# Trippasch/CudaRayTracer

Measured on AMD Instinct MI355X. Metric: Mray/s (and ms/frame) at 1920x1080, 64 spp, depth 8, random-spheres, higher is better.
Workload: dtype f32; 1 GPU; c2: 1920x1080, 64 spp, depth 8, RTIOW final random-spheres scene; width=1920, height=1080, spp=64, depth=8, parallelism=1 GPU, kernel_variant=-1

## Files before the change

### cudaraytracer_amd/_lib.py

```python
from __future__ import annotations

import ctypes as C
import os

from . import abi

LIB_PATH = _IN_TREE = os.path.join(os.path.dirname(os.path.abspath(__file__)), "librt_hip.so")
LIB_PATH = os.environ.get("RT_HIP_LIB", LIB_PATH)

EXPORTED = [
    "LaunchKernel",
    "LaunchRandInit",
    "LaunchRenderInit",
    "rt_last_error",
    "rt_version",
    "rt_abi_version",
    "rt_set_launch_flags",
    "rt_set_device",
    "rt_scene_create",
    "rt_scene_from_reference_graph",
    "rt_scene_update_materials",
    "rt_scene_destroy",
    "rt_scene_get_info",
    "rt_render_init",
# ... 34 lines not shown
    "rt_set_variant",
    "rt_set_tuning",
    "rt_glibc_srand",
    "rt_glibc_rand_next",
    "rt_builtin_scene",
    "rt_camera_inputs",
    "rt_procedural_texture",
    "rt_reference_graph_flatten",
    "rt_build_host_tables",
    "rt_tile_entries_host",
    "rt_set_tile_occlusion",
    "rt_tile_entries_device",
    "rt_set_bounce_entries",
    "rt_bounce_entries_host",
    "rt_bounce_entry_cells",
]

_lib = None


class RTError(RuntimeError):
    pass


def _declare(lib: C.CDLL) -> None:
    P = C.POINTER
    vp = C.c_void_p
    lib.rt_last_error.restype = C.c_char_p
    lib.rt_version.restype = C.c_char_p
    lib.rt_set_launch_flags.argtypes = [C.c_uint32]
# ... 58 lines not shown
                                               P(C.c_uint32), P(abi.ImageDesc), P(C.c_uint32)]
    lib.rt_build_host_tables.argtypes = [P(abi.SceneDesc), P(C.c_float), P(C.c_float), P(C.c_float),
                                         P(C.c_int32), P(abi.HostTablesInfo)]
    if LIB_PATH == _IN_TREE or hasattr(lib, "rt_tile_entries_host"):
        lib.rt_tile_entries_host.argtypes = [P(abi.SceneDesc), P(abi.InputStruct), C.c_uint32, C.c_uint32, P(abi.Tiling),
                                             C.c_uint32, C.c_uint32, C.c_uint32, P(C.c_uint32)]
    if LIB_PATH == _IN_TREE or hasattr(lib, "rt_set_tile_occlusion"):
        lib.rt_set_tile_occlusion.argtypes = [C.c_int]
        lib.rt_tile_entries_device.argtypes = [vp, P(abi.InputStruct), C.c_uint32, C.c_uint32, P(abi.Tiling), C.c_uint32,
                                               vp, vp]
    if LIB_PATH == _IN_TREE or hasattr(lib, "rt_set_bounce_entries"):
        lib.rt_set_bounce_entries.argtypes = [C.c_int]
        lib.rt_bounce_entries_host.argtypes = [P(abi.SceneDesc), P(C.c_float), P(C.c_float), P(C.c_uint32), P(C.c_uint32),
                                               P(C.c_uint16), P(abi.BounceEntriesInfo)]
        lib.rt_bounce_entry_cells.argtypes = [P(abi.BounceEntriesInfo), P(C.c_float), C.c_uint32, P(C.c_uint32)]
    lib.LaunchKernel.argtypes = [vp, C.c_uint, C.c_uint, C.c_uint, C.c_uint, vp, vp, abi.InputStruct]
    lib.LaunchKernel.restype = None
    lib.LaunchRandInit.argtypes = [vp]
    lib.LaunchRandInit.restype = None
    lib.LaunchRenderInit.argtypes = [abi.Dim3, abi.Dim3, C.c_uint, C.c_uint, vp]
    lib.LaunchRenderInit.restype = None


def lib() -> C.CDLL:
    global _lib
    if _lib is None:
        if not os.path.exists(LIB_PATH):
            raise RTError(f"{LIB_PATH} is missing: build it with `python -c 'import __graft_entry__ as g; g.build()'`")
        handle = C.CDLL(LIB_PATH)
        _declare(handle)
# ... 9 lines not shown
```

### cudaraytracer_amd/abi.py

```python
from __future__ import annotations

import ctypes as C

import numpy as np

RT_SPHERE, RT_XYRECT, RT_XZRECT, RT_YZRECT = 0, 1, 2, 3
RT_LAMBERTIAN, RT_METAL, RT_DIELECTRIC, RT_DIFFUSELIGHT = 0, 1, 2, 3
RT_CONSTANT, RT_CHECKER, RT_IMAGE = 0, 1, 2

RT_FLAG_FAITHFUL_GRID = 1 << 0
RT_FLAG_NO_STATE_WRITEBACK = 1 << 1
RT_FLAG_ACCUMULATE = 1 << 2
RT_FLAG_RIUS_LEFT_TO_RIGHT = 1 << 3
RT_FLAG_COUNT_TESTS = 1 << 4
RT_FLAG_RNG_PHILOX = 1 << 5
RT_FLAG_STATE_SOA = 1 << 6
RT_FLAG_ACCUMULATE_RESET = 1 << 7
RT_CAMERA_JITTER_PHILOX = 1 << 0
RT_DENOISE_DEMODULATE = 1 << 0
RT_DENOISE_COLOR_IS_SUM = 1 << 1
RT_TEMPORAL_COLOR_IS_SUM = 1 << 0
RT_TEMPORAL_RESET = 1 << 1
ABI_VERSION = 14
MOTION_NO_HISTORY = (0.0, 0.0, 0.0, 0.0)
# ... 318 lines not shown
        ("device_bytes", C.c_uint64),
    ]


class HostTablesInfo(C.Structure):
    _fields_ = [("num_nodes", C.c_uint32), ("num_prims", C.c_uint32), ("num_materials", C.c_uint32),
                ("depth", C.c_uint32)]


class BounceEntriesInfo(C.Structure):
    _fields_ = [("num_nodes", C.c_uint32), ("num_chain_nodes", C.c_uint32), ("num_records", C.c_uint32),
                ("depth", C.c_uint32), ("grid_dim", C.c_uint32 * 3), ("grid_origin", C.c_float * 3),
                ("grid_inv", C.c_float * 3), ("grid_off", C.c_float * 3)]


class GlibcRand(C.Structure):
    _fields_ = [("r", C.c_int32 * 34), ("idx", C.c_uint32)]


STATE_WORDS = 12
assert C.sizeof(CurandState) == 48
assert C.sizeof(InputStruct) == 72
assert C.sizeof(HittableDesc) == 40
assert C.sizeof(MaterialDesc) == 48
assert C.sizeof(TextureDesc) == 32


def make_inputs(origin, orientation, up, far_plane, near_plane, fov, bg_start, bg_end) -> InputStruct:
    s = InputStruct()
    s.origin[:] = [float(v) for v in origin]
# ... 13 lines not shown
```

### cudaraytracer_amd/csrc/api.cpp

```cpp
#include <hip/hip_runtime_api.h>

#include <algorithm>
#include <atomic>
#include <chrono>
#include <cmath>
#include <new>
#include <stdexcept>
#include <cstring>
#include <mutex>
#include <unordered_set>

#include "../../include/rt_reference_graph.h"
#include "rt_bounce_entry.h"
#include "rt_internal.h"
#include "rt_scene_device.h"

namespace rt {

static thread_local std::string g_last_error;

void set_error(const std::string& msg) { g_last_error = msg; }

template <class F>
static int guarded(const char* what, F&& f) {
// ... 33 lines not shown
    if (s->nodes48) (void)hipFree((void*)s->nodes48);
    if (s->refs) (void)hipFree((void*)s->refs);
    s->nodes48 = s->refs = nullptr;
    if (s->prims) (void)hipFree((void*)s->prims);
    if (s->prims_flat) (void)hipFree((void*)s->prims_flat);
    if (s->ref_nodes) (void)hipFree((void*)s->ref_nodes);
    if (s->flat_boxes) (void)hipFree((void*)s->flat_boxes);
    if (s->flat_ref_pairs) (void)hipFree((void*)s->flat_ref_pairs);
    s->prims_flat = s->ref_nodes = s->flat_boxes = s->flat_ref_pairs = nullptr;
    if (s->bvh_ref_nodes) (void)hipFree((void*)s->bvh_ref_nodes);
    if (s->bvh_boxes) (void)hipFree((void*)s->bvh_boxes);
    if (s->bvh_ref_pairs) (void)hipFree((void*)s->bvh_ref_pairs);
    s->bvh_ref_nodes = s->bvh_boxes = s->bvh_ref_pairs = nullptr;
    if (s->leaf_records) (void)hipFree((void*)s->leaf_records);
    if (s->bounce_grid) (void)hipFree((void*)s->bounce_grid);
    s->leaf_records = s->bounce_grid = nullptr;
    if (s->prim_source) (void)hipFree((void*)s->prim_source);
    if (s->flat_source) (void)hipFree((void*)s->flat_source);
    s->prim_source = s->flat_source = nullptr;
    if (s->mats) (void)hipFree((void*)s->mats);
    if (s->imgs) (void)hipFree((void*)s->imgs);
    s->nodes = s->prims = s->mats = nullptr;
    s->imgs = nullptr;
    s->texels = nullptr;
}

int create_device_scene(const HostScene& h, rt_scene** out, std::shared_ptr<void> shared_texels) {
    rt_scene* s = new rt_scene();
    s->host = h;
    s->host.texels = std::vector<uint8_t>();
    DeviceScene& d = s->dev;
// ... 19 lines not shown
    if ((rc = upload(h.flat_boxes, &p, "hipMalloc/hipMemcpy(flat_boxes)"))) goto fail;
    d.flat_boxes = p;
    if ((rc = upload(h.bvh_ref_nodes, &p, "hipMalloc/hipMemcpy(bvh_ref_nodes)"))) goto fail;
    d.bvh_ref_nodes = p;
    if ((rc = upload(h.bvh_boxes, &p, "hipMalloc/hipMemcpy(bvh_boxes)"))) goto fail;
    d.bvh_boxes = p;
    if ((rc = upload(h.bvh_ref_pairs, &p, "hipMalloc/hipMemcpy(bvh_ref_pairs)"))) goto fail;
    d.bvh_ref_pairs = p;
    d.flat_runs[0] = h.flat_runs[0];
    d.flat_runs[1] = h.flat_runs[1];
    if (!h.bounce_grid.empty()) {
        if ((rc = upload(h.leaf_records, &p, "hipMalloc/hipMemcpy(leaf_records)"))) goto fail;
        d.leaf_records = p;
        if ((rc = upload(h.bounce_grid, &p, "hipMalloc/hipMemcpy(bounce_grid)"))) goto fail;
        d.bounce_grid = p;
        for (int i = 0; i < 3; i++) {
            d.grid_dim[i] = h.grid_dim[i];
            d.grid_inv[i] = h.grid_inv[i];
            d.grid_off[i] = h.grid_off[i];
        }
    }
    if ((rc = upload(h.prim_source, &p, "hipMalloc/hipMemcpy(prim_source)"))) goto fail;
    d.prim_source = p;
    if ((rc = upload(h.flat_source, &p, "hipMalloc/hipMemcpy(flat_source)"))) goto fail;
    d.flat_source = p;
    if ((rc = upload(h.mats, &p, "hipMalloc/hipMemcpy(materials)"))) goto fail;
    d.mats = p;
    if ((rc = upload(h.imgs, &p, "hipMalloc/hipMemcpy(images)"))) goto fail;
    d.imgs = p;
    if (shared_texels) {
// ... 1 lines not shown
    } else {
        if ((rc = upload(h.texels, &p, "hipMalloc/hipMemcpy(texels)"))) goto fail;
        if (p) s->texel_block = std::shared_ptr<void>(p, [](void* q) { (void)hipFree(q); });
    }
    d.texels = s->texel_block.get();
    d.num_nodes = h.num_nodes;
    d.num_prims = h.num_prims;
    d.num_mats = h.num_mats;
    d.num_imgs = (uint32_t)(h.imgs.size() / 4);
    d.depth = h.depth;
    d.has_image_textures = h.has_image_textures;
    d.has_textures = h.has_textures;
    d.has_rects = h.has_rects;
    d.device_bytes = (h.nodes.size() + h.nodes48.size() + h.refs.size() + h.prims.size() + h.prims_flat.size() + h.ref_nodes.size() +
                      h.flat_boxes.size() + h.flat_ref_pairs.size() + h.bvh_ref_nodes.size() + h.bvh_boxes.size() + h.bvh_ref_pairs.size() + h.mats.size() +
                      h.prim_source.size() + h.flat_source.size() + h.leaf_records.size()) * 4 + h.bounce_grid.size() * 2 +
                     h.imgs.size() * 4 + h.texels.size();
    *out = s;
    return RT_OK;
fail:
    free_device(&d);
    delete s;
    return rc;
}

static void keep_description(rt_scene** scene, const rt_scene_desc& d, int texel_bytes) {
    static const uint8_t kHasData = 0;
    rt_scene* s = *scene;
    try {
        s->materials.assign(d.materials, d.materials + d.num_materials);
        s->images.assign(d.images, d.images + d.num_images);
// ... 121 lines not shown

struct ImageKey {
    const void* data;
    int32_t width, height;
    bool operator==(const ImageKey& o) const { return data == o.data && width == o.width && height == o.height; }
};

struct LaunchEntry {
    int device = 0;
    const void* world = nullptr;
    uint64_t last_use = 0;
    std::vector<rt_hittable_desc> hittables;
    std::vector<rt_material_desc> materials;
    std::vector<ImageKey> images;
    int texel_bytes = 0;
    std::shared_ptr<rt_scene> scene;
};

std::shared_ptr<rt_scene> own_scene(rt_scene* s, int device) {
    return std::shared_ptr<rt_scene>(s, [device](rt_scene* p) {
        int cur = 0;
        const bool restore = hipGetDevice(&cur) == hipSuccess;
        (void)hipSetDevice(device);
        rt_scene_destroy(p);
        if (restore) (void)hipSetDevice(cur);
    });
}

constexpr size_t kLaunchCacheEntries = 8;
std::mutex g_launch_mu;
// ... 24 lines not shown
        for (LaunchEntry& c : g_launch_cache)
            if (c.device == device && c.world == world) ent = &c;
        if (!ent) {
            if (g_launch_cache.size() >= kLaunchCacheEntries) {
                auto lru = std::min_element(g_launch_cache.begin(), g_launch_cache.end(),
                                            [](const LaunchEntry& a, const LaunchEntry& b) { return a.last_use < b.last_use; });
                g_launch_cache.erase(lru);
            }
            g_launch_cache.emplace_back();
            ent = &g_launch_cache.back();
            ent->device = device;
            ent->world = world;
        }
        ent->last_use = ++g_launch_clock;
        const bool geometry = !ent->scene || !same_bytes(ent->hittables, f.hittables) ||
                              ent->materials.size() != f.materials.size();
        const int texel_bytes = g_texel_bytes == 4 ? 4 : 3;
        const bool new_images = !ent->scene || !(ent->images == images) || ent->texel_bytes != texel_bytes;
        if (geometry || new_images) {
            rt_scene_desc d = f.desc();
            HostScene h;
            r = build_host_scene(&d, &h, &err, new_images);
            if (r) { set_error("LaunchKernel: " + err); return r; }
            rt_scene* fresh = nullptr;
            r = create_device_scene(h, &fresh, new_images ? nullptr : ent->scene->texel_block);
            if (r) return r;
            ent->scene = own_scene(fresh, device);
            ent->texel_bytes = texel_bytes;
        } else if (!same_bytes(ent->materials, f.materials)) {
            r = rt_scene_update_materials(ent->scene.get(), f.materials.data(), (uint32_t)f.materials.size());
            if (r) return r;
        }
        ent->hittables.swap(f.hittables);
        ent->materials.swap(f.materials);
        ent->images.swap(images);
        *out = ent->scene;
        return RT_OK;
    });
    if (host_ms) *host_ms = std::chrono::duration<double, std::milli>(std::chrono::steady_clock::now() - t0).count();
    return rc;
}

}
// ... 139 lines not shown
    });
    if (rc) return rc;
    std::memset(info, 0, sizeof(*info));
    info->num_nodes = h.num_nodes;
    info->depth = h.depth;
    if (h.bounce_grid.empty()) return RT_OK;
    info->num_chain_nodes = h.num_chain_nodes;
    info->num_records = (uint32_t)(h.leaf_records.size() / 4);
    for (int i = 0; i < 3; i++) {
        info->grid_dim[i] = h.grid_dim[i];
        info->grid_origin[i] = h.grid_origin[i];
        info->grid_inv[i] = h.grid_inv[i];
        info->grid_off[i] = h.grid_off[i];
    }
    if (chain_nodes) std::copy(h.chain_nodes.begin(), h.chain_nodes.end(), chain_nodes);
    if (nodes48) std::copy(h.nodes48.begin(), h.nodes48.end(), nodes48);
    if (refs) std::copy(h.refs.begin(), h.refs.end(), refs);
    if (records) std::copy(h.leaf_records.begin(), h.leaf_records.end(), records);
    if (grid) std::copy(h.bounce_grid.begin(), h.bounce_grid.end(), grid);
    return RT_OK;
}

int rt_bounce_entry_cells(const rt_bounce_entries_info* info, const float* origins, uint32_t n, uint32_t* cells) {
    if (!info || (n && (!origins || !cells))) { set_error("rt_bounce_entry_cells: NULL argument"); return RT_ERR_INVALID_ARGUMENT; }
    if (info->num_records == 0 || !info->grid_dim[0] || !info->grid_dim[1] || !info->grid_dim[2]) {
        set_error("rt_bounce_entry_cells: the scene has no bounce-entry table");
        return RT_ERR_INVALID_ARGUMENT;
    }
    const float dimf[3] = {(float)(info->grid_dim[0] - 1u), (float)(info->grid_dim[1] - 1u), (float)(info->grid_dim[2] - 1u)};
    for (uint32_t i = 0; i < n; i++)
        cells[i] = bounce_cell(origins[3 * (size_t)i], origins[3 * (size_t)i + 1], origins[3 * (size_t)i + 2], info->grid_inv,
                               info->grid_off, dimf, info->grid_dim);
    return RT_OK;
}

static TemporalCamera temporal_camera(const rt_input_struct& in) {
    TemporalCamera c;
    const float* up = in.up;
    const float* fw = in.orientation;
    const float cx = up[1] * fw[2] - up[2] * fw[1];
    const float cy = -(up[0] * fw[2] - up[2] * fw[0]);
    const float cz = up[0] * fw[1] - up[1] * fw[0];
    const float inv = 1.0f / std::sqrt((cx * cx + cy * cy) + cz * cz);
    c.right[0] = inv * cx;
    c.right[1] = inv * cy;
    c.right[2] = inv * cz;
    c.fov = in.fov;
// ... 232 lines not shown
```

### cudaraytracer_amd/csrc/render.hip

```cpp
#include <hip/hip_runtime.h>

#include <cfloat>
#include <cstdio>
#include <cstdlib>
#include <cstring>
#include <atomic>
#include <map>
#include <numeric>
#include <memory>
#include <mutex>
#include <tuple>
#include <type_traits>
#include <vector>

#include "rt_epilogue.h"
#include "rt_internal.h"
#include "rt_scene_device.h"
#include "rt_tile_entry.h"

namespace rt {
namespace dev {

struct f3 {
    float x, y, z;
};

enum NodeLayout { NODES_48 = 0, NODES_64 = 2 };
__device__ __forceinline__ f3 mk(float x, float y, float z) { return f3{x, y, z}; }
__device__ __forceinline__ f3 add(f3 a, f3 b) { return mk(a.x + b.x, a.y + b.y, a.z + b.z); }
__device__ __forceinline__ f3 sub(f3 a, f3 b) { return mk(a.x - b.x, a.y - b.y, a.z - b.z); }
__device__ __forceinline__ f3 mulv(f3 a, f3 b) { return mk(a.x * b.x, a.y * b.y, a.z * b.z); }
__device__ __forceinline__ f3 scale(float t, f3 v) { return mk(t * v.x, t * v.y, t * v.z); }
// ... 170 lines not shown
    uint32_t prefetch_stop;
    uint32_t group_tiles;
    uint32_t queue_base;
    uint32_t group_perm_a;
    uint32_t group_perm_b, group_perm_k;
    uint32_t queue_host_reset;
    uint32_t linger_ticks;
    uint32_t group_chunk;
    const uint4* tile_entries;
    uint32_t camera_resolve;
    uint32_t path_end_step;
    const uint4* bounce_records;
    const uint16_t* bounce_grid;
    float grid_inv[3], grid_off[3];
    float grid_max[3];
    uint32_t grid_nx, grid_ny;
};

constexpr int kStackMax = 64;
constexpr int kBlock = 256;
constexpr uint32_t kQueueCounters = 16;
constexpr uint32_t kQueueSlotWords = kQueueCounters + 3;
static_assert(kQueueCounters >= 1 && kQueueCounters <= 32, "queue heads");
constexpr uint32_t kQueueAllDone = kQueueCounters == 32 ? 0xffffffffu : (1u << kQueueCounters) - 1u;

enum StackKind { STACK_SCRATCH = 0, STACK_LDS = 1, STACK_LDS16 = 3, STACK_NONE = 4 };

struct ScratchStack {
    int s[kStackMax];
    int n;
    __device__ __forceinline__ void init(uint32_t*) { n = 0; }
// ... 1225 lines not shown
                const uint32_t e[6] = {ry & 0xffffu, ry >> 16, rz & 0xffffu, rz >> 16, rw & 0xffffu, rw >> 16};
                uint32_t n = 0;
#pragma unroll
                for (int i = 0; i < 6; i++)
                    if (e[i] != kTileEntryNone) {
                        stk[(kStackBase + i) * 64] = (typename RefW<WIDE>::Entry)e[i];
                        n = (uint32_t)i + 1u;
                    }
                c.sp = kStackBase + n;
            }
        }
    }
}

template <bool WIDE>
__device__ __forceinline__ void v3_bounce_entry(KParamsC* q, typename RefW<WIDE>::Entry* const stk, const f3 ro, Cursor& c) {
    if constexpr (!WIDE) {
        const uint4* const recs = q->bounce_records;
        if (!recs) return;
        const float fx = fminf(fmaxf(__builtin_fmaf(ro.x, q->grid_inv[0], q->grid_off[0]), 0.0f), q->grid_max[0]);
        const float fy = fminf(fmaxf(__builtin_fmaf(ro.y, q->grid_inv[1], q->grid_off[1]), 0.0f), q->grid_max[1]);
        const float fz = fminf(fmaxf(__builtin_fmaf(ro.z, q->grid_inv[2], q->grid_off[2]), 0.0f), q->grid_max[2]);
        const uint32_t cell = ((uint32_t)fz * q->grid_ny + (uint32_t)fy) * q->grid_nx + (uint32_t)fx;
        const uint4 r = recs[q->bounce_grid[cell]];
        const uint32_t e0 = r.x & 0xffffu;
        if (e0 != kTileEntryRoot) {
            c.leaf = (int)e0;
            c.node = (int)(r.x >> 16);
            const uint32_t e[6] = {r.y & 0xffffu, r.y >> 16, r.z & 0xffffu, r.z >> 16, r.w & 0xffffu, r.w >> 16};
            uint32_t n = 0;
#pragma unroll
            for (int i = 0; i < 6; i++) n += e[i] != kTileEntryNone ? 1u : 0u;
#pragma unroll
            for (int i = 0; i < 6; i++)
                if ((uint32_t)i < n) stk[(kStackBase + n - 1u - (uint32_t)i) * 64] = (typename RefW<WIDE>::Entry)e[i];
            c.sp = kStackBase + n;
        }
    }
}
// ... 641 lines not shown
                    c.mode = MODE_ENDED;
                } else if (ended) {
                    col = mk(__uint_as_float(park[(PK_COL + 0) * 64]), __uint_as_float(park[(PK_COL + 1) * 64]),
                             __uint_as_float(park[(PK_COL + 2) * 64]));
                    v3_next_sample<WIDE>(P, x, g, contrib, rng, col, att, sample, depth, ro, rd, c, rays, tile, stk);
                    park[(PK_COL + 0) * 64] = __float_as_uint(col.x);
                    park[(PK_COL + 1) * 64] = __float_as_uint(col.y);
                    park[(PK_COL + 2) * 64] = __float_as_uint(col.z);
                } else {
                    v3_start_trace<WIDE>(P.num_nodes, c, rays);
                    bounce = true;
                    if (COUNT_TESTS && P.ray_dump) dump_ray(P, depth == P.ray_dump_depth, ro, rd);
                }
                v3_park<COMPACT, false>(park, rng, col, att, sample, depth, rays);
            }
            if (bounce) v3_bounce_entry<WIDE>(kparams_reload(), stk, ro, c);
            if (!RT_REPLAY_SAME_PASS || __ballot(c.mode == MODE_REPLAY) == 0u) break;
            bvh_replay_wave(kparams_reload(), prims, c, ro, rd, cnt, COUNT_TESTS);
        }
        if constexpr (kItemsBuild) {
            const uint64_t needm = __ballot(c.mode == MODE_NEED);
            if (items && needm != 0) {
                const uint32_t item = next_item +
                    __builtin_amdgcn_mbcnt_hi((uint32_t)(needm >> 32), __builtin_amdgcn_mbcnt_lo((uint32_t)needm, 0u));
                next_item += (uint32_t)__popcll(needm);
                if (c.mode == MODE_NEED) {
                    if (item < n_items) {
                        const uint32_t p = item & 63u;
                        const uint32_t bx = tile % P.tiles_x, by = tile / P.tiles_x;
                        const uint32_t px = bx * 8u + (p & 7u), pg = global_row(P, by * 8u + (p >> 3));
                        R rng = begin_rng<R>(nullptr, 0u, pg * P.width + px);
// ... 2669 lines not shown
                           (const float*)S.prims, F, E.rec, P.num_tiles);
        rc = hip_check(hipGetLastError(), "rt_render: tile entry kernel launch", RT_ERR_LAUNCH);
        if (rc != RT_OK) return rc;
        E.filled = true;
        E.scene_uid = S.uid;
        E.frame = F;
    }
    P.tile_entries = (const uint4*)E.rec;
    P.camera_resolve = g_camera_resolve == 1 ? kCameraResolveCap : (uint32_t)g_camera_resolve;
    P.path_end_step = (uint32_t)g_path_end_step;
    return RT_OK;
}

void bind_bounce_entries(dev::KParams& P, const int kernel, const DeviceScene& S) {
    if (kernel != 3 || S.wide_refs || !g_bounce_entries || !S.leaf_records || !S.bounce_grid) return;
    P.bounce_records = (const uint4*)S.leaf_records;
    P.bounce_grid = (const uint16_t*)S.bounce_grid;
    for (int i = 0; i < 3; i++) {
        P.grid_inv[i] = S.grid_inv[i];
        P.grid_off[i] = S.grid_off[i];
        P.grid_max[i] = (float)(S.grid_dim[i] - 1u);
    }
    P.grid_nx = S.grid_dim[0];
    P.grid_ny = S.grid_dim[1];
}

void fill_kernel_params(dev::KParams& P, const Variant& V, const LaunchShape& L, const DeviceScene& S) {
    P.lds_wave_words = L.wave_words;
    if (V.kernel == 5 || V.kernel == 6) fill_flat_tables(P, S);
    const int rius_trips = V.kernel == 6 ? g_rius_trips_persistent : g_rius_trips;
    P.rius_cap = rius_trips > 0 ? (uint32_t)rius_trips : 0xffffffffu;
    const uint32_t tile = V.block == 64 ? 8u : 16u;
    P.tiles_x = (P.width + tile - 1) / tile;
    P.num_tiles = P.tiles_x * ((P.local_rows + tile - 1) / tile);
}

// ... 182 lines not shown
```

### cudaraytracer_amd/csrc/rt_bounce_entry.h

```cpp
#pragma once

#include <cmath>
#include <cstdint>

#include "rt_tile_entry.h"

namespace rt {

constexpr uint32_t kBounceGridMaxCells = 4096;
constexpr uint32_t kBounceChainMax = 7;

RT_TILE_HD inline uint32_t bounce_cell(const float x, const float y, const float z, const float* inv, const float* off,
                                       const float* dimf, const uint32_t* dim) {
    const float fx = fminf(fmaxf(fmaf(x, inv[0], off[0]), 0.0f), dimf[0]);
    const float fy = fminf(fmaxf(fmaf(y, inv[1], off[1]), 0.0f), dimf[1]);
    const float fz = fminf(fmaxf(fmaf(z, inv[2], off[2]), 0.0f), dimf[2]);
    return ((uint32_t)fz * dim[1] + (uint32_t)fy) * dim[0] + (uint32_t)fx;
}

}
```

### cudaraytracer_amd/csrc/rt_internal.h

```cpp
#pragma once

#include <cstdint>
#include <string>
#include <vector>

#include "../../include/rt_hip.h"

namespace rt {

constexpr int kLeafMax = 4;
constexpr uint32_t kOccupancyDepth = 12;
extern thread_local int g_leaf_max;
extern thread_local int g_sah_traversal_x10;
extern thread_local int g_texel_bytes;
constexpr int kRegStackDepth = 24;
constexpr uint32_t kFlatMaxPrims = 64;
constexpr uint32_t kRefTreeMaxDepth = 14;
constexpr uint32_t kRefTreeMaxDepthBvh = 31;

struct HostScene {
    std::vector<float> nodes;
    std::vector<float> nodes48;
    std::vector<uint32_t> refs;
    bool wide_refs = false;
// ... 14 lines not shown
    std::vector<float> ref_nodes;
    std::vector<float> flat_ref_pairs;
    std::vector<float> flat_boxes;
    uint32_t flat_runs[2] = {0u, 0u};
    std::vector<float> bvh_ref_nodes;
    std::vector<float> bvh_boxes;
    std::vector<float> bvh_ref_pairs;
    uint32_t num_chain_nodes = 0;
    std::vector<float> chain_nodes;
    std::vector<uint32_t> leaf_records;
    std::vector<uint16_t> bounce_grid;
    uint32_t grid_dim[3] = {0u, 0u, 0u};
    float grid_origin[3] = {0.0f, 0.0f, 0.0f};
    float grid_inv[3] = {0.0f, 0.0f, 0.0f};
    float grid_off[3] = {0.0f, 0.0f, 0.0f};
};

int build_host_scene(const rt_scene_desc* desc, HostScene* out, std::string* err, bool with_texels = true);

int pack_materials(const rt_material_desc* mats, uint32_t n, uint32_t num_images, std::vector<float>* out,
                   std::string* err);

struct FlatDesc {
    std::vector<rt_hittable_desc> hittables;
    std::vector<rt_material_desc> materials;
    std::vector<rt_image_desc> images;
    rt_scene_desc desc() const {
        rt_scene_desc d;
        d.hittables = hittables.data();
        d.num_hittables = (uint32_t)hittables.size();
        d.materials = materials.data();
// ... 69 lines not shown
```

### cudaraytracer_amd/csrc/rt_scene_device.h

```cpp
#pragma once

#include <cstdint>
#include <memory>

#include "rt_internal.h"

namespace rt {

struct DeviceScene {
    const void* nodes = nullptr;
    const void* nodes48 = nullptr;
    const void* refs = nullptr;
    bool wide_refs = false;
    const void* prims = nullptr;
    const void* prims_flat = nullptr;
    const void* ref_nodes = nullptr;
    const void* flat_ref_pairs = nullptr;
    const void* flat_boxes = nullptr;
    const void* bvh_ref_nodes = nullptr;
    const void* bvh_boxes = nullptr;
    const void* bvh_ref_pairs = nullptr;
    uint32_t flat_runs[2] = {0u, 0u};
    const void* prim_source = nullptr;
    const void* flat_source = nullptr;
    const void* leaf_records = nullptr;
    const void* bounce_grid = nullptr;
    uint32_t grid_dim[3] = {0u, 0u, 0u};
    float grid_inv[3] = {0.0f, 0.0f, 0.0f}, grid_off[3] = {0.0f, 0.0f, 0.0f};
    const void* mats = nullptr;
    const void* imgs = nullptr;
    const void* texels = nullptr;
    uint32_t num_nodes = 0, num_prims = 0, num_mats = 0, depth = 0;
    uint32_t num_imgs = 0;
    bool has_image_textures = false;
    bool has_textures = false;
    bool has_rects = false;
    uint64_t device_bytes = 0;
    uint64_t uid = 0;
};

int create_device_scene(const HostScene& h, rt_scene** out, std::shared_ptr<void> shared_texels = nullptr);
// ... 17 lines not shown
```

### cudaraytracer_amd/csrc/scene_build.cpp

```cpp
#include <algorithm>
#include <limits>
#include <functional>
#include <array>
#include <cmath>
#include <cstring>
#include <numeric>

#include "rt_bounce_entry.h"
#include "rt_internal.h"

namespace rt {
namespace {

struct Box {
    float lo[3], hi[3];
    void empty() {
        for (int i = 0; i < 3; i++) { lo[i] = INFINITY; hi[i] = -INFINITY; }
    }
    void grow(const Box& b) {
        for (int i = 0; i < 3; i++) { lo[i] = std::min(lo[i], b.lo[i]); hi[i] = std::max(hi[i], b.hi[i]); }
    }
    float area() const {
        float dx = hi[0] - lo[0], dy = hi[1] - lo[1], dz = hi[2] - lo[2];
        if (!(dx >= 0) || !(dy >= 0) || !(dz >= 0)) return 0.0f;
        return 2.0f * (dx * dy + dy * dz + dz * dx);
    }
// ... 342 lines not shown
                    float d2 = 0.0f;
                    for (int i = 0; i < 3; i++) {
                        const float d = std::max(std::max(b.lo[i] - c[i], c[i] - b.hi[i]), 0.0f);
                        d2 += d * d;
                    }
                    const float area = b.area();
                    if (d2 < best_dist || (d2 == best_dist && area < best_area)) {
                        best = l;
                        best_dist = d2;
                        best_area = area;
                    }
                }
                out->bounce_grid[((size_t)z * dim[1] + y) * dim[0] + x] = (uint16_t)best;
            }

    out->num_chain_nodes = (uint32_t)chain.size();
    out->chain_nodes.resize(chain.size() * 16);
    out->nodes48.resize((size_t)(N + chain.size()) * 12);
    out->refs.resize((size_t)N + chain.size());
    for (size_t i = 0; i < chain.size(); i++) {
        pack_node16(chain[i], out->chain_nodes.data() + i * 16);
        pack_node48(chain[i], false, out->nodes48.data() + (N + i) * 12);
        out->refs[N + i] = ((uint32_t)chain[i].child[0] & 0xffffu) | ((uint32_t)chain[i].child[1] << 16);
    }
    out->leaf_records.resize(records.size() * 4);
    for (size_t i = 0; i < records.size(); i++)
        for (int w = 0; w < 4; w++) out->leaf_records[4 * i + w] = records[i][2 * w] | (records[i][2 * w + 1] << 16);
}

struct RefNode {
    float lo[3], hi[3];
    int child[2];
    uint32_t depth;
};
void ref_prim_box(const rt_hittable_desc& h, float lo[3], float hi[3]) {
    if (h.type == RT_SPHERE) {
// ... 393 lines not shown
```

### cudaraytracer_amd/renderer.py

```python
from __future__ import annotations

import ctypes as C

import numpy as np
import torch

from . import abi
from ._lib import RTError, check, lib
from .scenes import Scene


class DeviceScene:

    def __init__(self, scene: Scene | None = None, reference_graph: int | None = None):
        L = lib()
        self.handle = C.c_void_p()
        self.scene = scene
        if reference_graph is not None:
            check(L.rt_scene_from_reference_graph(C.c_void_p(reference_graph), C.byref(self.handle)),
                  "rt_scene_from_reference_graph")
        else:
            self._desc = scene.desc()
            check(L.rt_scene_create(C.byref(self._desc), C.byref(self.handle)), "rt_scene_create")

# ... 103 lines not shown
            lib().rt_scene_destroy(self.handle)
            self.handle = C.c_void_p()

    def __del__(self):
        try:
            self.close()
        except Exception:
            pass


def set_tile_occlusion(on: bool) -> bool:
    prev = lib().rt_set_tile_occlusion(1 if on else 0)
    if prev < 0:
        check(prev, "rt_set_tile_occlusion")
    return bool(prev)


def camera_rays(inputs: abi.InputStruct, width: int, height: int, pixels=None, jitter=(0.5, 0.5), sample: int = 0,
                seed: int = 1984, frame: int = 0, tiling: abi.Tiling | None = None, device=None):
    if pixels is not None and not isinstance(pixels, torch.Tensor):
        pixels = torch.from_numpy(np.array(pixels, dtype=np.int64).astype(np.uint32).view(np.int32)).cuda()
    if pixels is not None:
        if pixels.dtype not in (torch.int32, torch.uint32) or pixels.dim() != 1 or not pixels.is_cuda:
            raise ValueError("pixels must be a 32-bit integer (n,) tensor on the device")
        pixels = pixels.contiguous()
        device = pixels.device
    elif device is None:
        device = torch.device("cuda", torch.cuda.current_device())
    t = tiling if tiling is not None else abi.Tiling(max(height, 1), 1, 0, height)
    n = pixels.shape[0] if pixels is not None else t.local_rows * width
# ... 335 lines not shown
```

### include/rt_hip.h

```cpp
#ifndef RT_HIP_H
#define RT_HIP_H

#include <stddef.h>
#include <stdint.h>

#ifdef __cplusplus
extern "C" {
#endif

typedef enum rt_status {
    RT_OK = 0,
    RT_ERR_INVALID_ARGUMENT = -1,
    RT_ERR_INVALID_SCENE = -2,
    RT_ERR_OUT_OF_MEMORY = -3,
    RT_ERR_DEVICE = -4,
    RT_ERR_LAUNCH = -5,
    RT_ERR_UNSUPPORTED = -6
} rt_status;

typedef enum rt_hittable_type {
    RT_SPHERE = 0,
    RT_XYRECT = 1,
    RT_XZRECT = 2,
    RT_YZRECT = 3
// ... 427 lines not shown
                           const rt_tiling* tiling, uint32_t flags, void* records, rt_stream stream);

int rt_set_bounce_entries(int on);

typedef struct rt_bounce_entries_info {
    uint32_t num_nodes, num_chain_nodes, num_records, depth;
    uint32_t grid_dim[3];
    float grid_origin[3];
    float grid_inv[3];
    float grid_off[3];
} rt_bounce_entries_info;
int rt_bounce_entries_host(const rt_scene_desc* desc, float* chain_nodes, float* nodes48, uint32_t* refs,
                           uint32_t* records, uint16_t* grid, rt_bounce_entries_info* info);
int rt_bounce_entry_cells(const rt_bounce_entries_info* info, const float* origins, uint32_t n, uint32_t* cells);

typedef struct rt_glibc_rand { int32_t r[34]; uint32_t idx; } rt_glibc_rand;
void rt_glibc_srand(rt_glibc_rand* g, uint32_t seed);
int32_t rt_glibc_rand_next(rt_glibc_rand* g);

int rt_builtin_scene(int which, uint32_t seed, rt_hittable_desc* hittables, uint32_t* num_hittables,
                     rt_material_desc* materials, uint32_t* num_materials);

int rt_procedural_texture(int kind, int32_t width, int32_t height, uint8_t* rgb);

void rt_camera_inputs(const float position[3], const float orientation[3], const float world_up[3],
                      float fov_degrees, float near_plane, float far_plane, const float bg_start[3],
                      const float bg_end[3], rt_input_struct* out);

#ifdef __cplusplus
}
// ... 4 lines not shown
```

Baseline: 34950 Mray/s.

## Add direction-classed bounce entry records to prune unreachable BVH siblings

Extends the bounce-entry grid so each grid record has 25 variants, keyed by the secondary ray's dominant axis and octant, plus a fallback class. On the host, sibling subtrees along the leaf path that a ray in a given direction class cannot reach from the record's region are dropped, and new chain nodes are built from the remaining pairs. The goal is to shorten the restart stack for secondary bounces and so skip box tests. In exchange, each bounce entry now computes the direction class, the record table is 25 times larger, scene build does more work, and the conservative reachability test must stay correct.

Result: faster. 35660 Mray/s (median of 6 runs) (+2.0%).

```diff
diff --git a/cudaraytracer_amd/_lib.py b/cudaraytracer_amd/_lib.py
--- a/cudaraytracer_amd/_lib.py
+++ b/cudaraytracer_amd/_lib.py
@@ -72,6 +72,8 @@
     "rt_set_bounce_entries",
     "rt_bounce_entries_host",
     "rt_bounce_entry_cells",
+    "rt_set_bounce_classes",
+    "rt_bounce_class_entries_host",
 ]
 
 _lib = None
@@ -160,6 +162,11 @@
         lib.rt_bounce_entries_host.argtypes = [P(abi.SceneDesc), P(C.c_float), P(C.c_float), P(C.c_uint32), P(C.c_uint32),
                                                P(C.c_uint16), P(abi.BounceEntriesInfo)]
         lib.rt_bounce_entry_cells.argtypes = [P(abi.BounceEntriesInfo), P(C.c_float), C.c_uint32, P(C.c_uint32)]
+    if LIB_PATH == _IN_TREE or hasattr(lib, "rt_set_bounce_classes"):
+        lib.rt_set_bounce_classes.argtypes = [C.c_int]
+        lib.rt_bounce_class_entries_host.argtypes = [P(abi.SceneDesc), C.c_int, C.c_uint32, P(C.c_uint32), P(C.c_float),
+                                                     P(C.c_uint32), P(C.c_double), P(C.c_float), P(C.c_float), C.c_uint32,
+                                                     P(C.c_uint32), P(abi.BounceClassInfo)]
     lib.LaunchKernel.argtypes = [vp, C.c_uint, C.c_uint, C.c_uint, C.c_uint, vp, vp, abi.InputStruct]
     lib.LaunchKernel.restype = None
     lib.LaunchRandInit.argtypes = [vp]
diff --git a/cudaraytracer_amd/abi.py b/cudaraytracer_amd/abi.py
--- a/cudaraytracer_amd/abi.py
+++ b/cudaraytracer_amd/abi.py
@@ -356,6 +356,15 @@
                 ("grid_inv", C.c_float * 3), ("grid_off", C.c_float * 3)]
 
 
+BOUNCE_CLASSES = 25
+BOUNCE_CLASS_FULL = 24
+
+
+class BounceClassInfo(C.Structure):
+    _fields_ = [("form", C.c_uint32), ("num_records", C.c_uint32), ("num_class_nodes", C.c_uint32),
+                ("first_class_node", C.c_uint32)]
+
+
 class GlibcRand(C.Structure):
     _fields_ = [("r", C.c_int32 * 34), ("idx", C.c_uint32)]
 
diff --git a/cudaraytracer_amd/csrc/api.cpp b/cudaraytracer_amd/csrc/api.cpp
--- a/cudaraytracer_amd/csrc/api.cpp
+++ b/cudaraytracer_amd/csrc/api.cpp
@@ -71,7 +71,8 @@
     s->bvh_ref_nodes = s->bvh_boxes = s->bvh_ref_pairs = nullptr;
     if (s->leaf_records) (void)hipFree((void*)s->leaf_records);
     if (s->bounce_grid) (void)hipFree((void*)s->bounce_grid);
-    s->leaf_records = s->bounce_grid = nullptr;
+    if (s->class_records) (void)hipFree((void*)s->class_records);
+    s->leaf_records = s->bounce_grid = s->class_records = nullptr;
     if (s->prim_source) (void)hipFree((void*)s->prim_source);
     if (s->flat_source) (void)hipFree((void*)s->flat_source);
     s->prim_source = s->flat_source = nullptr;
@@ -121,6 +122,8 @@
         d.leaf_records = p;
         if ((rc = upload(h.bounce_grid, &p, "hipMalloc/hipMemcpy(bounce_grid)"))) goto fail;
         d.bounce_grid = p;
+        if ((rc = upload(h.class_records, &p, "hipMalloc/hipMemcpy(class_records)"))) goto fail;
+        d.class_records = p;
         for (int i = 0; i < 3; i++) {
             d.grid_dim[i] = h.grid_dim[i];
             d.grid_inv[i] = h.grid_inv[i];
@@ -152,7 +155,7 @@
     d.has_rects = h.has_rects;
     d.device_bytes = (h.nodes.size() + h.nodes48.size() + h.refs.size() + h.prims.size() + h.prims_flat.size() + h.ref_nodes.size() +
                       h.flat_boxes.size() + h.flat_ref_pairs.size() + h.bvh_ref_nodes.size() + h.bvh_boxes.size() + h.bvh_ref_pairs.size() + h.mats.size() +
-                      h.prim_source.size() + h.flat_source.size() + h.leaf_records.size()) * 4 + h.bounce_grid.size() * 2 +
+                      h.prim_source.size() + h.flat_source.size() + h.leaf_records.size() + h.class_records.size()) * 4 + h.bounce_grid.size() * 2 +
                      h.imgs.size() * 4 + h.texels.size();
     *out = s;
     return RT_OK;
@@ -304,6 +307,7 @@
     std::vector<rt_material_desc> materials;
     std::vector<ImageKey> images;
     int texel_bytes = 0;
+    int bounce_classes = 0;
     std::shared_ptr<rt_scene> scene;
 };
 
@@ -358,7 +362,7 @@
         }
         ent->last_use = ++g_launch_clock;
         const bool geometry = !ent->scene || !same_bytes(ent->hittables, f.hittables) ||
-                              ent->materials.size() != f.materials.size();
+                              ent->materials.size() != f.materials.size() || ent->bounce_classes != g_bounce_classes;
         const int texel_bytes = g_texel_bytes == 4 ? 4 : 3;
         const bool new_images = !ent->scene || !(ent->images == images) || ent->texel_bytes != texel_bytes;
         if (geometry || new_images) {
@@ -371,6 +375,7 @@
             if (r) return r;
             ent->scene = own_scene(fresh, device);
             ent->texel_bytes = texel_bytes;
+            ent->bounce_classes = g_bounce_classes;
         } else if (!same_bytes(ent->materials, f.materials)) {
             r = rt_scene_update_materials(ent->scene.get(), f.materials.data(), (uint32_t)f.materials.size());
             if (r) return r;
@@ -540,8 +545,9 @@
         info->grid_off[i] = h.grid_off[i];
     }
     if (chain_nodes) std::copy(h.chain_nodes.begin(), h.chain_nodes.end(), chain_nodes);
-    if (nodes48) std::copy(h.nodes48.begin(), h.nodes48.end(), nodes48);
-    if (refs) std::copy(h.refs.begin(), h.refs.end(), refs);
+    const size_t total = (size_t)h.num_nodes + h.num_chain_nodes;
+    if (nodes48) std::copy(h.nodes48.begin(), h.nodes48.begin() + total * 12, nodes48);
+    if (refs) std::copy(h.refs.begin(), h.refs.begin() + total, refs);
     if (records) std::copy(h.leaf_records.begin(), h.leaf_records.end(), records);
     if (grid) std::copy(h.bounce_grid.begin(), h.bounce_grid.end(), grid);
     return RT_OK;
@@ -557,6 +563,64 @@
     for (uint32_t i = 0; i < n; i++)
         cells[i] = bounce_cell(origins[3 * (size_t)i], origins[3 * (size_t)i + 1], origins[3 * (size_t)i + 2], info->grid_inv,
                                info->grid_off, dimf, info->grid_dim);
+    return RT_OK;
+}
+
+int rt_set_bounce_classes(int form) {
+    if (form < 0 || form > 2) {
+        set_error("rt_set_bounce_classes: the value must be 0, 1 or 2");
+        return RT_ERR_INVALID_ARGUMENT;
+    }
+    const int prev = g_bounce_classes;
+    g_bounce_classes = form;
+    return prev;
+}
+
+int rt_bounce_class_entries_host(const rt_scene_desc* desc, int form, uint32_t node_limit, uint32_t* records,
+                                 float* class_nodes48, uint32_t* class_refs, double* regions, const float* origins,
+                                 const float* directions, uint32_t n, uint32_t* classes, rt_bounce_class_info* info) {
+    if (!info) { set_error("rt_bounce_class_entries_host: info is NULL"); return RT_ERR_INVALID_ARGUMENT; }
+    if (form < -1 || form > 2) { set_error("rt_bounce_class_entries_host: form must be -1, 0, 1 or 2"); return RT_ERR_INVALID_ARGUMENT; }
+    if (node_limit > 0x7fffu) { set_error("rt_bounce_class_entries_host: node_limit must be at most 0x7fff"); return RT_ERR_INVALID_ARGUMENT; }
+    if (n && (!directions || !classes)) { set_error("rt_bounce_class_entries_host: NULL directions or classes"); return RT_ERR_INVALID_ARGUMENT; }
+    HostScene h;
+    const int prev_form = g_bounce_classes;
+    const uint32_t prev_limit = g_bounce_class_node_limit;
+    if (form >= 0) g_bounce_classes = form;
+    if (node_limit) g_bounce_class_node_limit = node_limit;
+    int rc = guarded("rt_bounce_class_entries_host", [&]() -> int {
+        std::string err;
+        int r = build_host_scene(desc, &h, &err);
+        if (r) set_error("rt_bounce_class_entries_host: " + err);
+        return r;
+    });
+    g_bounce_classes = prev_form;
+    g_bounce_class_node_limit = prev_limit;
+    if (rc) return rc;
+    std::memset(info, 0, sizeof(*info));
+    info->num_records = (uint32_t)(h.leaf_records.size() / 4);
+    info->form = h.bounce_classes;
+    info->num_class_nodes = h.num_class_nodes;
+    info->first_class_node = h.num_nodes + h.num_chain_nodes;
+    if (h.bounce_classes) {
+        if (records) std::copy(h.class_records.begin(), h.class_records.end(), records);
+        const size_t first = info->first_class_node;
+        if (class_nodes48) std::copy(h.nodes48.begin() + first * 12, h.nodes48.end(), class_nodes48);
+        if (class_refs) std::copy(h.refs.begin() + first, h.refs.end(), class_refs);
+        if (regions) std::copy(h.class_regions.begin(), h.class_regions.end(), regions);
+    }
+    if (n) {
+        if (h.bounce_grid.empty()) {
+            set_error("rt_bounce_class_entries_host: the scene has no bounce-entry table");
+            return RT_ERR_INVALID_ARGUMENT;
+        }
+        const float dims[3] = {(float)h.grid_dim[0], (float)h.grid_dim[1], (float)h.grid_dim[2]};
+        const float zero[3] = {0.0f, 0.0f, 0.0f};
+        for (uint32_t i = 0; i < n; i++)
+            classes[i] = origins ? bounce_class_at(origins + 3 * (size_t)i, directions + 3 * (size_t)i, h.grid_inv, h.grid_off, dims)
+                                 : bounce_class(directions[3 * (size_t)i], directions[3 * (size_t)i + 1],
+                                                directions[3 * (size_t)i + 2], zero[0], zero[1], zero[2]);
+    }
     return RT_OK;
 }
 
diff --git a/cudaraytracer_amd/csrc/render.hip b/cudaraytracer_amd/csrc/render.hip
--- a/cudaraytracer_amd/csrc/render.hip
+++ b/cudaraytracer_amd/csrc/render.hip
@@ -16,6 +16,7 @@
 #include "rt_epilogue.h"
 #include "rt_internal.h"
 #include "rt_scene_device.h"
+#include "rt_bounce_entry.h"
 #include "rt_tile_entry.h"
 
 namespace rt {
@@ -216,7 +217,9 @@
     const uint16_t* bounce_grid;
     float grid_inv[3], grid_off[3];
     float grid_max[3];
+    float grid_dims[3];
     uint32_t grid_nx, grid_ny;
+    uint32_t bounce_classes;
 };
 
 constexpr int kStackMax = 64;
@@ -1472,15 +1475,24 @@
 }
 
 template <bool WIDE>
-__device__ __forceinline__ void v3_bounce_entry(KParamsC* q, typename RefW<WIDE>::Entry* const stk, const f3 ro, Cursor& c) {
+__device__ __forceinline__ void v3_bounce_entry(KParamsC* q, typename RefW<WIDE>::Entry* const stk, const f3 ro, const f3 rd,
+                                                Cursor& c) {
     if constexpr (!WIDE) {
         const uint4* const recs = q->bounce_records;
         if (!recs) return;
-        const float fx = fminf(fmaxf(__builtin_fmaf(ro.x, q->grid_inv[0], q->grid_off[0]), 0.0f), q->grid_max[0]);
-        const float fy = fminf(fmaxf(__builtin_fmaf(ro.y, q->grid_inv[1], q->grid_off[1]), 0.0f), q->grid_max[1]);
-        const float fz = fminf(fmaxf(__builtin_fmaf(ro.z, q->grid_inv[2], q->grid_off[2]), 0.0f), q->grid_max[2]);
+        const float ux = __builtin_fmaf(ro.x, q->grid_inv[0], q->grid_off[0]);
+        const float uy = __builtin_fmaf(ro.y, q->grid_inv[1], q->grid_off[1]);
+        const float uz = __builtin_fmaf(ro.z, q->grid_inv[2], q->grid_off[2]);
+        const float fx = fminf(fmaxf(ux, 0.0f), q->grid_max[0]);
+        const float fy = fminf(fmaxf(uy, 0.0f), q->grid_max[1]);
+        const float fz = fminf(fmaxf(uz, 0.0f), q->grid_max[2]);
         const uint32_t cell = ((uint32_t)fz * q->grid_ny + (uint32_t)fy) * q->grid_nx + (uint32_t)fx;
-        const uint4 r = recs[q->bounce_grid[cell]];
+        uint32_t rec = q->bounce_grid[cell];
+        if (q->bounce_classes)
+            rec = rec * kBounceClasses + bounce_class(rd.x, rd.y, rd.z, ux - fminf(fmaxf(ux, 0.0f), q->grid_dims[0]),
+                                                      uy - fminf(fmaxf(uy, 0.0f), q->grid_dims[1]),
+                                                      uz - fminf(fmaxf(uz, 0.0f), q->grid_dims[2]));
+        const uint4 r = recs[rec];
         const uint32_t e0 = r.x & 0xffffu;
         if (e0 != kTileEntryRoot) {
             c.leaf = (int)e0;
@@ -2152,7 +2164,7 @@
                 }
                 v3_park<COMPACT, false>(park, rng, col, att, sample, depth, rays);
             }
-            if (bounce) v3_bounce_entry<WIDE>(kparams_reload(), stk, ro, c);
+            if (bounce) v3_bounce_entry<WIDE>(kparams_reload(), stk, ro, rd, c);
             if (!RT_REPLAY_SAME_PASS || __ballot(c.mode == MODE_REPLAY) == 0u) break;
             bvh_replay_wave(kparams_reload(), prims, c, ro, rd, cnt, COUNT_TESTS);
         }
@@ -4852,12 +4864,14 @@
 
 void bind_bounce_entries(dev::KParams& P, const int kernel, const DeviceScene& S) {
     if (kernel != 3 || S.wide_refs || !g_bounce_entries || !S.leaf_records || !S.bounce_grid) return;
-    P.bounce_records = (const uint4*)S.leaf_records;
+    P.bounce_classes = g_bounce_classes && S.class_records ? 1u : 0u;
+    P.bounce_records = (const uint4*)(P.bounce_classes ? S.class_records : S.leaf_records);
     P.bounce_grid = (const uint16_t*)S.bounce_grid;
     for (int i = 0; i < 3; i++) {
         P.grid_inv[i] = S.grid_inv[i];
         P.grid_off[i] = S.grid_off[i];
         P.grid_max[i] = (float)(S.grid_dim[i] - 1u);
+        P.grid_dims[i] = (float)S.grid_dim[i];
     }
     P.grid_nx = S.grid_dim[0];
     P.grid_ny = S.grid_dim[1];
diff --git a/cudaraytracer_amd/csrc/rt_bounce_entry.h b/cudaraytracer_amd/csrc/rt_bounce_entry.h
--- a/cudaraytracer_amd/csrc/rt_bounce_entry.h
+++ b/cudaraytracer_amd/csrc/rt_bounce_entry.h
@@ -18,4 +18,30 @@
     return ((uint32_t)fz * dim[1] + (uint32_t)fy) * dim[0] + (uint32_t)fx;
 }
 
+constexpr uint32_t kBounceClasses = 25;
+constexpr uint32_t kBounceClassFull = 24;
+
+RT_TILE_HD inline uint32_t bounce_class(const float dx, const float dy, const float dz, const float ex, const float ey,
+                                        const float ez) {
+    const float ax = fabsf(dx), ay = fabsf(dy), az = fabsf(dz);
+    const uint32_t k = ax >= ay ? (ax >= az ? 0u : 2u) : (ay >= az ? 1u : 2u);
+    uint32_t bx, by, bz;
+    __builtin_memcpy(&bx, &dx, 4);
+    __builtin_memcpy(&by, &dy, 4);
+    __builtin_memcpy(&bz, &dz, 4);
+    const uint32_t cls = k * 8u + ((bx >> 31) | (by >> 31) << 1 | (bz >> 31) << 2);
+    const bool ok = fminf(fminf(ax, ay), az) > 0.0f && (ax + ay) + az < INFINITY && (fabsf(ex) + fabsf(ey)) + fabsf(ez) <= 1.0f;
+    return ok ? cls : kBounceClassFull;
 }
+
+RT_TILE_HD inline uint32_t bounce_class_at(const float* o, const float* d, const float* inv, const float* off,
+                                           const float* dims) {
+    float e[3];
+    for (int i = 0; i < 3; i++) {
+        const float u = fmaf(o[i], inv[i], off[i]);
+        e[i] = u - fminf(fmaxf(u, 0.0f), dims[i]);
+    }
+    return bounce_class(d[0], d[1], d[2], e[0], e[1], e[2]);
+}
+
+}
diff --git a/cudaraytracer_amd/csrc/rt_internal.h b/cudaraytracer_amd/csrc/rt_internal.h
--- a/cudaraytracer_amd/csrc/rt_internal.h
+++ b/cudaraytracer_amd/csrc/rt_internal.h
@@ -52,7 +52,14 @@
     float grid_origin[3] = {0.0f, 0.0f, 0.0f};
     float grid_inv[3] = {0.0f, 0.0f, 0.0f};
     float grid_off[3] = {0.0f, 0.0f, 0.0f};
+    uint32_t bounce_classes = 0;
+    uint32_t num_class_nodes = 0;
+    std::vector<uint32_t> class_records;
+    std::vector<double> class_regions;
 };
+
+extern thread_local int g_bounce_classes;
+extern thread_local uint32_t g_bounce_class_node_limit;
 
 int build_host_scene(const rt_scene_desc* desc, HostScene* out, std::string* err, bool with_texels = true);
 
diff --git a/cudaraytracer_amd/csrc/rt_scene_device.h b/cudaraytracer_amd/csrc/rt_scene_device.h
--- a/cudaraytracer_amd/csrc/rt_scene_device.h
+++ b/cudaraytracer_amd/csrc/rt_scene_device.h
@@ -25,6 +25,7 @@
     const void* flat_source = nullptr;
     const void* leaf_records = nullptr;
     const void* bounce_grid = nullptr;
+    const void* class_records = nullptr;
     uint32_t grid_dim[3] = {0u, 0u, 0u};
     float grid_inv[3] = {0.0f, 0.0f, 0.0f}, grid_off[3] = {0.0f, 0.0f, 0.0f};
     const void* mats = nullptr;
diff --git a/cudaraytracer_amd/csrc/scene_build.cpp b/cudaraytracer_amd/csrc/scene_build.cpp
--- a/cudaraytracer_amd/csrc/scene_build.cpp
+++ b/cudaraytracer_amd/csrc/scene_build.cpp
@@ -1,5 +1,6 @@
 #include <algorithm>
 #include <limits>
+#include <map>
 #include <functional>
 #include <array>
 #include <cmath>
@@ -9,7 +10,15 @@
 #include "rt_bounce_entry.h"
 #include "rt_internal.h"
 
+#ifndef RT_BOUNCE_CLASSES_DEFAULT
+#define RT_BOUNCE_CLASSES_DEFAULT 2
+#endif
+
 namespace rt {
+
+thread_local int g_bounce_classes = RT_BOUNCE_CLASSES_DEFAULT;
+thread_local uint32_t g_bounce_class_node_limit = 0x7fffu;
+
 namespace {
 
 struct Box {
@@ -382,12 +391,148 @@
                 out->bounce_grid[((size_t)z * dim[1] + y) * dim[0] + x] = (uint16_t)best;
             }
 
-    out->num_chain_nodes = (uint32_t)chain.size();
-    out->chain_nodes.resize(chain.size() * 16);
+    const size_t num_chain = chain.size();
+    bool flat_axis = false;
+    for (int i = 0; i < 3; i++) flat_axis = flat_axis || !(out->grid_inv[i] > 0.0f);
+    if (g_bounce_classes != 0 && !flat_axis) {
+        const size_t R = records.size();
+        std::vector<double>& reg = out->class_regions;
+        reg.resize(R * 6);
+        for (size_t r = 0; r < R; r++)
+            for (int i = 0; i < 3; i++) { reg[6 * r + i] = INFINITY; reg[6 * r + 3 + i] = -INFINITY; }
+        for (uint32_t z = 0; z < dim[2]; z++)
+            for (uint32_t y = 0; y < dim[1]; y++)
+                for (uint32_t x = 0; x < dim[0]; x++) {
+                    const uint32_t cell[3] = {x, y, z};
+                    double* q = reg.data() + 6 * (size_t)out->bounce_grid[((size_t)z * dim[1] + y) * dim[0] + x];
+                    for (int i = 0; i < 3; i++) {
+                        const double inv = (double)out->grid_inv[i], off = (double)out->grid_off[i];
+                        const double lo = ((cell[i] == 0 ? -1.0 : (double)cell[i]) - off) / inv;
+                        const double hi = ((cell[i] + 1u == dim[i] ? (double)dim[i] + 1.0 : (double)cell[i] + 1.0) - off) / inv;
+                        q[i] = std::min(q[i], lo);
+                        q[3 + i] = std::max(q[3 + i], hi);
+                    }
+                }
+        std::vector<signed char> span_node(N, -1);
+        std::function<bool(int)> spans = [&](const int ref) -> bool {
+            if (ref < 0) {
+                if (!any) return true;
+                const uint32_t r = ~(uint32_t)ref, first = r >> 2, count = (r & 3u) + 1u;
+                for (uint32_t i = first; i < first + count; i++)
+                    if (spanning(B.prims[B.order[i]])) return true;
+                return false;
+            }
+            if (span_node[ref] < 0) {
+                const bool a = spans(B.nodes[ref].child[0]), b = spans(B.nodes[ref].child[1]);
+                span_node[ref] = a || b;
+            }
+            return span_node[ref] != 0;
+        };
+        const auto reachable = [](const double* Rg, const Box& S, const uint32_t cls) -> bool {
+            const uint32_t k = cls >> 3;
+            double D = 0.0, A = 0.0;
+            for (int j = 0; j < 3; j++) {
+                const double slo = (double)S.lo[j], shi = (double)S.hi[j], rlo = Rg[j], rhi = Rg[3 + j];
+                D += (rhi > shi ? rhi : shi) - (rlo < slo ? rlo : slo);
+                double a = rlo < 0.0 ? -rlo : rlo;
+                const double b = rhi < 0.0 ? -rhi : rhi, c = slo < 0.0 ? -slo : slo, d = shi < 0.0 ? -shi : shi;
+                a = a > b ? a : b;
+                a = a > c ? a : c;
+                A += a > d ? a : d;
+            }
+            const double m = 0x1p-8 * D + 0x1p-18 * A;
+            if (!(m - m == 0.0)) return true;
+            const bool neg_k = (cls >> k & 1u) != 0;
+            const double s = neg_k ? Rg[3 + k] - (double)S.lo[k] : (double)S.hi[k] - Rg[k];
+            if (s < -m) return false;
+            for (uint32_t j = 0; j < 3; j++) {
+                if (j == k) continue;
+                const bool neg = (cls >> j & 1u) != 0;
+                const double lo = neg ? Rg[j] - s - m : Rg[j], hi = neg ? Rg[3 + j] : Rg[3 + j] + s + m;
+                if ((double)S.hi[j] < lo - m || (double)S.lo[j] > hi + m) return false;
+            }
+            return true;
+        };
+        std::vector<uint32_t>& cr = out->class_records;
+        for (uint32_t form = (uint32_t)g_bounce_classes;; form = 1) {
+            chain.resize(num_chain);
+            cr.assign(R * kBounceClasses * 4, 0u);
+            std::map<std::pair<int, int>, int> pair_id;
+            for (size_t i = 0; i < num_chain; i++) pair_id[{chain[i].child[0], chain[i].child[1]}] = (int)(N + i);
+            for (size_t l = 0; l < R; l++) {
+                const Leaf& L = leaves[l];
+                const size_t a = L.path.size();
+                const double* Rg = reg.data() + 6 * l;
+                const bool whole = records[l][0] == kTileEntryRoot || !(Rg[0] <= Rg[3]);
+                const auto sib_ref = [&](const size_t i) { return B.nodes[L.path[i].node].child[1 - L.path[i].side]; };
+                const auto sib_box = [&](const size_t i) -> const Box& { return B.nodes[L.path[i].node].box[1 - L.path[i].side]; };
+                for (uint32_t cls = 0; cls < kBounceClasses; cls++) {
+                    std::array<uint32_t, kTileEntryMax> e = records[l];
+                    if (!whole && cls != kBounceClassFull) {
+                        std::vector<char> reach(a);
+                        for (size_t i = 0; i < a; i++) reach[i] = spans(sib_ref(i)) || reachable(Rg, sib_box(i), cls);
+                        std::vector<int> refs;
+                        if (form == 1) {
+                            if ((a & 1u) && reach[a - 1]) refs.push_back(sib_ref(a - 1));
+                            for (size_t k = a / 2; k >= 1; k--)
+                                if (reach[2 * k - 1] || reach[2 * k - 2])
+                                    refs.push_back(chain_of[(size_t)L.path[2 * k - 1].node * 2 + (size_t)L.path[2 * k - 1].side]);
+                        } else {
+                            std::vector<size_t> kept;
+                            for (size_t i = 0; i < a; i++)
+                                if (reach[i]) kept.push_back(i);
+                            if (kept.size() & 1u) refs.push_back(sib_ref(kept.back()));
+                            for (size_t k = kept.size() / 2; k >= 1; k--) {
+                                const size_t lo = kept[2 * k - 1], up = kept[2 * k - 2];
+                                int& id = pair_id[{sib_ref(lo), sib_ref(up)}];
+                                if (id == 0) {
+                                    id = (int)(N + chain.size());
+                                    Builder::Node c;
+                                    c.child[0] = sib_ref(lo);
+                                    c.box[0] = sib_box(lo);
+                                    c.child[1] = sib_ref(up);
+                                    c.box[1] = sib_box(up);
+                                    chain.push_back(c);
+                                }
+                                refs.push_back(id);
+                            }
+                        }
+                        const size_t m = refs.size();
+                        bool fits = m <= kBounceChainMax && (m == 0 || m - 1 <= out->depth);
+                        for (size_t j = 0; j < m && fits; j++) {
+                            const uint32_t h = (uint32_t)(m - 1 - j);
+                            uint32_t top = 0;
+                            if (refs[j] >= (int)N) {
+                                const Builder::Node& c = chain[(size_t)refs[j] - N];
+                                top = h + 1u + std::max(ref_height(c.child[0]), ref_height(c.child[1]));
+                            } else if (refs[j] >= 0) {
+                                top = h + height[refs[j]];
+                            }
+                            fits = top <= out->depth;
+                        }
+                        if (fits) {
+                            e.fill(kTileEntryNone);
+                            e[0] = (uint32_t)L.ref & 0xffffu;
+                            for (size_t j = 0; j < m; j++) e[1 + j] = (uint32_t)refs[j] & 0xffffu;
+                        }
+                    }
+                    uint32_t* w = cr.data() + (l * kBounceClasses + cls) * 4;
+                    for (int i = 0; i < 4; i++) w[i] = e[2 * i] | (e[2 * i + 1] << 16);
+                }
+            }
+            if (form == 2 && N + chain.size() >= g_bounce_class_node_limit) continue;
+            out->bounce_classes = form;
+            break;
+        }
+        out->num_class_nodes = (uint32_t)(chain.size() - num_chain);
+    }
+
+    out->num_chain_nodes = (uint32_t)num_chain;
+    out->chain_nodes.resize(num_chain * 16);
     out->nodes48.resize((size_t)(N + chain.size()) * 12);
     out->refs.resize((size_t)N + chain.size());
     for (size_t i = 0; i < chain.size(); i++) {
-        pack_node16(chain[i], out->chain_nodes.data() + i * 16);
+        if (i < num_chain) pack_node16(chain[i], out->chain_nodes.data() + i * 16);
         pack_node48(chain[i], false, out->nodes48.data() + (N + i) * 12);
         out->refs[N + i] = ((uint32_t)chain[i].child[0] & 0xffffu) | ((uint32_t)chain[i].child[1] << 16);
     }
diff --git a/cudaraytracer_amd/renderer.py b/cudaraytracer_amd/renderer.py
--- a/cudaraytracer_amd/renderer.py
+++ b/cudaraytracer_amd/renderer.py
@@ -141,6 +141,13 @@
     if prev < 0:
         check(prev, "rt_set_tile_occlusion")
     return bool(prev)
+
+
+def set_bounce_classes(form: int) -> int:
+    prev = lib().rt_set_bounce_classes(int(form))
+    if prev < 0:
+        check(prev, "rt_set_bounce_classes")
+    return prev
 
 
 def camera_rays(inputs: abi.InputStruct, width: int, height: int, pixels=None, jitter=(0.5, 0.5), sample: int = 0,
diff --git a/include/rt_hip.h b/include/rt_hip.h
--- a/include/rt_hip.h
+++ b/include/rt_hip.h
@@ -465,6 +465,15 @@
                            uint32_t* records, uint16_t* grid, rt_bounce_entries_info* info);
 int rt_bounce_entry_cells(const rt_bounce_entries_info* info, const float* origins, uint32_t n, uint32_t* cells);
 
+int rt_set_bounce_classes(int form);
+
+typedef struct rt_bounce_class_info {
+    uint32_t form, num_records, num_class_nodes, first_class_node;
+} rt_bounce_class_info;
+int rt_bounce_class_entries_host(const rt_scene_desc* desc, int form, uint32_t node_limit, uint32_t* records,
+                                 float* class_nodes48, uint32_t* class_refs, double* regions, const float* origins,
+                                 const float* directions, uint32_t n, uint32_t* classes, rt_bounce_class_info* info);
+
 typedef struct rt_glibc_rand { int32_t r[34]; uint32_t idx; } rt_glibc_rand;
 void rt_glibc_srand(rt_glibc_rand* g, uint32_t seed);
 int32_t rt_glibc_rand_next(rt_glibc_rand* g);
```
